# snakers4/mnasnet-pytorch

Hardware: AMD Instinct MI355X
Metric: images/sec MNASNet-1.0 224^2 bf16 train step (higher is better)
Workload: dtype bf16

## Files before the change

### mnasnet_pytorch_amd/csrc/mnas_tcx.hip

```cpp
#include "mnas_common.h"

struct TcxArgs {
    int M2;
    int Ho, Wo, Co, Ci;
    int Kpad;
    int rows_pad;
    int cib;
    float rcp_hw, rcp_wo;
    const uint16_t* dy;
    const uint16_t* w;
    void* out;
    float* stats;
    const void* red_y;
    const float* red_bn;
};

__device__ __forceinline__ int tcx_fdiv(int n, int d, float rcp) {
    if (rcp == 0.f) return n / d;
    int q = (int)((float)n * rcp);
    const int r = n - q * d;
    q += (r >= d) ? 1 : 0;
    q -= (r < 0) ? 1 : 0;
    return q;
}

template <int TPW, int KSM>
__global__ __launch_bounds__(256) void k_tcx(TcxArgs a) {
    extern __shared__ __attribute__((aligned(16))) unsigned char smem[];
    constexpr int WC = TPW * 16, SP = WC + 8;
    uint16_t* stage = (uint16_t*)smem;
    float* lds_rc = (float*)(stage + 4 * 16 * SP);
    float* lds_fin = lds_rc + 4 * WC;
    const int tid = threadIdx.x, lane = tid & 63;
    const int cls = __builtin_amdgcn_readfirstlane(tid >> 6);
    const int ph = cls >> 1, pw = cls & 1;
    const int l15 = lane & 15, lg = lane >> 4;
    const int ci0 = blockIdx.y * a.cib;
    const int cin = min(a.cib, a.Ci - ci0);
    const bool do_red = a.red_y != nullptr;
    const int nslots = (1 + ph) * (1 + pw);
    const int kc = nslots * a.Co;

    if (do_red)
        for (int i = tid; i < 4 * WC; i += 256) {
            const int r = i / WC, c = i - r * WC, cc = ci0 + c;
            float v = 0.f;
            if (c < cin) {
                if (r == 0) v = a.red_bn[cc];
                else if (r == 1) v = a.red_bn[a.Ci + cc];
                else if (r == 2) v = a.red_bn[6 * a.Ci + cc];
                else v = -a.red_bn[5 * a.Ci + cc] * a.red_bn[6 * a.Ci + cc];
            }
            lds_rc[i] = v;
        }
    int koff[KSM];
    unsigned nbits = 0;
    bf16x8_t wf[TPW][KSM];
#pragma unroll
    for (int ks = 0; ks < KSM; ++ks) {
        const int k = ks * 32 + lg * 8;
        const int slot = k / a.Co, co = k - slot * a.Co;
        const bool kok = k < kc;
        int dh = 0, dw = 0;
        if (kok) {
            if (ph && pw) { dh = slot >> 1; dw = slot & 1; }
            else if (ph) dh = slot;
            else if (pw) dw = slot;
        }
        koff[ks] = kok ? (dh * a.Wo + dw) * a.Co + co : -1;
        nbits |= (unsigned)(dh | (dw << 1)) << (2 * ks);
        const int col = (dh * 2 + dw) * a.Co + co;
#pragma unroll
        for (int t = 0; t < TPW; ++t) {
            const int rl = t * 16 + l15;
            const int row = cls * a.Ci + ci0 + rl;
            uint4 v = make_uint4(0, 0, 0, 0);
            if (kok && rl < cin && row < a.rows_pad) v = *(const uint4*)(a.w + (size_t)row * a.Kpad + col);
            wf[t][ks] = *(const bf16x8_t*)&v;
        }
    }
    if (do_red) __syncthreads();

    uint16_t* st = stage + cls * 16 * SP;
    const int hw = a.Ho * a.Wo;
    const int ngroups = (a.M2 + 15) >> 4;
    const int cpp = cin >> 3;
    constexpr int NPASS = (16 * (WC / 8) + 63) / 64;
    float r1[NPASS][8], r2[NPASS][8];
#pragma unroll
    for (int p = 0; p < NPASS; ++p)
#pragma unroll
        for (int j = 0; j < 8; ++j) { r1[p][j] = 0.f; r2[p][j] = 0.f; }

    uint4 v0[KSM];
    int ooff[NPASS], ooff_n[NPASS];
    uint4 yv[NPASS], yv_n[NPASS];
    auto issue = [&](int g) {
        const int m = g * 16 + l15;
        const bool mok = m < a.M2;
        const int n = mok ? tcx_fdiv(m, hw, a.rcp_hw) : 0, rem = m - n * hw;
        const int i = mok ? tcx_fdiv(rem, a.Wo, a.rcp_wo) : 0, j = rem - i * a.Wo;
        const uint16_t* base = a.dy + (size_t)(mok ? m : 0) * a.Co;
#pragma unroll
        for (int ks = 0; ks < KSM; ++ks) {
            const int dh = (nbits >> (2 * ks)) & 1, dw = (nbits >> (2 * ks + 1)) & 1;
            v0[ks] = make_uint4(0, 0, 0, 0);
            if (mok && koff[ks] >= 0 && i + dh < a.Ho && j + dw < a.Wo) v0[ks] = *(const uint4*)(base + koff[ks]);
        }
#pragma unroll
        for (int p = 0; p < NPASS; ++p) {
            const int q = p * 64 + lane;
            const int px = q / cpp, ch = q - px * cpp;
            const int mm = g * 16 + px;
            ooff_n[p] = -1;
            yv_n[p] = make_uint4(0, 0, 0, 0);
            if (q < 16 * cpp && mm < a.M2) {
                const int n2 = tcx_fdiv(mm, hw, a.rcp_hw), rem2 = mm - n2 * hw;
                const int i2 = tcx_fdiv(rem2, a.Wo, a.rcp_wo), j2 = rem2 - i2 * a.Wo;
                ooff_n[p] = ((n2 * 2 * a.Ho + 2 * i2 + ph) * (2 * a.Wo) + 2 * j2 + pw) * a.Ci + ci0 + ch * 8;
                if (do_red) yv_n[p] = *(const uint4*)((const uint16_t*)a.red_y + ooff_n[p]);
            }
        }
    };
    if ((int)blockIdx.x < ngroups) issue(blockIdx.x);
    for (int g = blockIdx.x; g < ngroups; g += gridDim.x) {
        const int m0 = g * 16;
        bf16x8_t bf[KSM];
#pragma unroll
        for (int ks = 0; ks < KSM; ++ks) bf[ks] = *(const bf16x8_t*)&v0[ks];
#pragma unroll
        for (int p = 0; p < NPASS; ++p) { ooff[p] = ooff_n[p]; yv[p] = yv_n[p]; }
        if (g + (int)gridDim.x < ngroups) issue(g + gridDim.x);
#pragma unroll
        for (int t = 0; t < TPW; ++t) {
            f32x4_t acc = (f32x4_t){0.f, 0.f, 0.f, 0.f};
#pragma unroll
            for (int ks = 0; ks < KSM; ++ks) acc = __builtin_amdgcn_mfma_f32_16x16x32_bf16(wf[t][ks], bf[ks], acc, 0, 0, 0);
            uint2 pk;
            pk.x = pack_bf16(acc[0], acc[1]);
            pk.y = pack_bf16(acc[2], acc[3]);
            *(uint2*)(st + l15 * SP + t * 16 + lg * 4) = pk;
        }
        __builtin_amdgcn_wave_barrier();
#pragma unroll
        for (int p = 0; p < NPASS; ++p) {
            const int q = p * 64 + lane;
            const int px = q / cpp, ch = q - px * cpp;
            if (ooff[p] >= 0) {
                const uint4 pk = *(const uint4*)(st + px * SP + ch * 8);
                st_u4((uint16_t*)a.out + ooff[p], pk, true);
                if (do_red) {
                    const uint32_t gu[4] = {pk.x, pk.y, pk.z, pk.w}, yu[4] = {yv[p].x, yv[p].y, yv[p].z, yv[p].w};
                    const int cl = ch * 8;
#pragma unroll
                    for (int jj = 0; jj < 4; ++jj)
                        mnas_red2(gu[jj], yu[jj], mnas_ld2(lds_rc + cl + 2 * jj), mnas_ld2(lds_rc + WC + cl + 2 * jj),
                                  mnas_ld2(lds_rc + 2 * WC + cl + 2 * jj), mnas_ld2(lds_rc + 3 * WC + cl + 2 * jj), &r1[p][2 * jj], &r2[p][2 * jj]);
                }
            }
        }
        __builtin_amdgcn_wave_barrier();
    }
    if (do_red && a.stats) {
        float* outp = a.stats;
        for (int p = 0; p < NPASS; ++p) {
            __syncthreads();
#pragma unroll
            for (int j = 0; j < 8; ++j) { lds_fin[tid * 16 + j] = r1[p][j]; lds_fin[tid * 16 + 8 + j] = r2[p][j]; }
            __syncthreads();
            for (int i = tid; i < 2 * cin; i += 256) {
                const int r = i / cin, c = i - r * cin, cc = c >> 3, j = c & 7;
                float v = 0.f;
                for (int th = 0; th < 256; ++th)
                    if (((p * 64 + (th & 63)) % cpp) == cc && p * 64 + (th & 63) < 16 * cpp) v += lds_fin[th * 16 + r * 8 + j];
                float* d = outp + ((size_t)r * a.Ci + ci0 + c) * gridDim.x + blockIdx.x;
                *d = (p == 0 ? 0.f : *d) + v;
            }
        }
    }
}

struct TcxPlan { int tpw, ksm, cib, nblocks; size_t lds; };

int mnas_tcx_enabled() {
    static int on = -1;
    if (on < 0) on = mnas_diag_env("MNAS_TCX", 1);
    return on;
}
static bool tcx_plan(int Ho, int Wo, int Co, int Ci, TcxPlan* p) {
    if (!mnas_tcx_enabled() || (Co & 7) || (Ci & 7) || Co < 8 || Ci < 8 || Ho < 1 || Wo < 1) return false;
    const int ksm = (4 * Co + 31) / 32;
    if (Ci <= 16 && ksm <= 3) { p->tpw = 1; p->ksm = 3; }
    else if (Ci <= 32 && ksm <= 5) { p->tpw = 2; p->ksm = 5; }
    else return false;
    p->cib = p->tpw * 16 < Ci ? p->tpw * 16 : Ci;
    p->nblocks = (Ci + p->cib - 1) / p->cib;
    const int wc = p->tpw * 16;
    p->lds = (size_t)4 * 16 * (wc + 8) * 2 + (size_t)4 * wc * 4 + (size_t)256 * 16 * 4;
    return true;
}
int mnas_tcx_ok(int Ho, int Wo, int Co, int Ci) {
    TcxPlan p;
    return tcx_plan(Ho, Wo, Co, Ci, &p) ? 1 : 0;
}
int mnas_tcx_parts(int N, int Ho, int Wo, int Co, int Ci) {
    TcxPlan p;
    if (!tcx_plan(Ho, Wo, Co, Ci, &p)) return -1;
    if ((long long)N * Ho * Wo * 4 * Ci > 0x7fffffff) return -1;
    const long long groups = ((long long)N * Ho * Wo + 15) / 16;
    static int wgs = -1;
    if (wgs < 0) wgs = mnas_diag_env("MNAS_TCX_WGS", 0);
    int want = (wgs > 0 ? wgs : (p.tpw == 1 ? 1024 : 768)) / p.nblocks;
    if (want < 64) want = 64;
    return (int)(groups < want ? groups : want);
}

int mnas_tcx_dgrad(const MnasTconvDgrad* c, void* stream) {
    TcxPlan p;
    const long long M2 = (long long)c->N * c->Ho * c->Wo;
    if (M2 * 4 * c->Ci > 0x7fffffff || !tcx_plan(c->Ho, c->Wo, c->Co, c->Ci, &p)) return MNAS_EINVAL;
    TcxArgs a;
    a.M2 = (int)M2; a.Ho = c->Ho; a.Wo = c->Wo; a.Co = c->Co; a.Ci = c->Ci;
    a.Kpad = (4 * c->Co + 31) / 32 * 32; a.rows_pad = (4 * c->Ci + 15) / 16 * 16; a.cib = p.cib;
    a.rcp_hw = M2 < (1 << 24) ? 1.0f / (float)(c->Ho * c->Wo) : 0.f;
    a.rcp_wo = M2 < (1 << 24) ? 1.0f / (float)c->Wo : 0.f;
    a.dy = (const uint16_t*)c->dy; a.w = (const uint16_t*)c->w; a.out = c->out; a.stats = c->stats;
    a.red_y = c->red_y; a.red_bn = c->red_bn;
    hipStream_t s = (hipStream_t)stream;
#define MNAS_TCX(T_, K_) \
    if (p.tpw == T_ && p.ksm == K_) { \
        hipLaunchKernelGGL((k_tcx<T_, K_>), dim3(c->nparts, p.nblocks), dim3(256), p.lds, s, a); \
        MNAS_CHECK_LAUNCH(); \
        return MNAS_OK; \
    }
    MNAS_TCX(1, 3) MNAS_TCX(2, 5)
#undef MNAS_TCX
    return MNAS_EINVAL;
}

struct TcrArgs {
    int N, Ho, Wo, Co, Ci;
    int Kpad, rows_pad;
    int LW, Cp;
    const uint16_t* dy;
    const uint16_t* w;
    void* out;
    float* stats;
    const void* red_y;
    const float* red_bn;
};

template <int KQ0, int KQ1, int KQ3>
__global__ __launch_bounds__(512) void k_tcr(TcrArgs a) {
    extern __shared__ __attribute__((aligned(16))) unsigned char smem[];
    constexpr int NB = 16, PPW = NB + 4, NSLOT = 256, MAXS = 6;
    constexpr int KQ[4] = {KQ0, KQ1, KQ1, KQ3};
    const int tid = threadIdx.x, lane = tid & 63;
    const int wave = __builtin_amdgcn_readfirstlane(tid >> 6);
    const int kq = wave & 3, phalf = wave >> 2;
    const int l15 = lane & 15, lg = lane >> 4;
    const int img_elems = ((a.Ho + 1) * a.LW * a.Cp + 7) & ~7;
    uint16_t* img = (uint16_t*)smem;
    float* part = (float*)(img + img_elems);
    float* lds_rc = part + 4 * NSLOT * PPW;
    float* lds_fin = part;
    const int ci0 = blockIdx.y * NB;
    const bool do_red = a.red_y != nullptr;
    const int npc = a.Ho * a.Wo;

    for (int i = tid; i < img_elems >> 3; i += 512) ((uint4*)img)[i] = make_uint4(0, 0, 0, 0);
    if (do_red)
        for (int i = tid; i < 4 * NB; i += 512) {
            const int r = i / NB, cc = ci0 + i % NB;
            float v = 0.f;
            if (cc < a.Ci) {
                if (r == 0) v = a.red_bn[cc];
                else if (r == 1) v = a.red_bn[a.Ci + cc];
                else if (r == 2) v = a.red_bn[6 * a.Ci + cc];
                else v = -a.red_bn[5 * a.Ci + cc] * a.red_bn[6 * a.Ci + cc];
            }
            lds_rc[i] = v;
        }
    bf16x8_t wf0[KQ0], wf1[KQ1], wf2[KQ1], wf3[KQ3];
    int to0[KQ0], to1[KQ1], to2[KQ1], to3[KQ3];
    auto load_class = [&](auto& wf, auto& to, int cls, int kqn) {
        const int ph = cls >> 1, pw = cls & 1;
        const int kc = (1 + ph) * (1 + pw) * a.Co;
#pragma unroll
        for (int j = 0; j < kqn; ++j) {
            const int k = (kq + 4 * j) * 32 + lg * 8;
            const bool kok = k < kc;
            const int slot = kok ? k / a.Co : 0, co = kok ? k - slot * a.Co : 0;
            int dh = 0, dw = 0;
            if (ph && pw) { dh = slot >> 1; dw = slot & 1; }
            else if (ph) dh = slot;
            else if (pw) dw = slot;
            to[j] = kok ? (dh * a.LW + dw) * a.Cp + co : -1;
            const int row = cls * a.Ci + ci0 + l15, col = (dh * 2 + dw) * a.Co + co;
            uint4 v = make_uint4(0, 0, 0, 0);
            if (kok && ci0 + l15 < a.Ci && row < a.rows_pad) v = *(const uint4*)(a.w + (size_t)row * a.Kpad + col);
            wf[j] = *(const bf16x8_t*)&v;
        }
    };
    load_class(wf0, to0, 0, KQ0); load_class(wf1, to1, 1, KQ1); load_class(wf2, to2, 2, KQ1); load_class(wf3, to3, 3, KQ3);
    int pbase[2];
#pragma unroll
    for (int t = 0; t < 2; ++t) {
        const int p = (phalf * 2 + t) * 16 + l15;
        const int pp = p < npc ? p : 0;
        const int i = pp / a.Wo, j = pp - i * a.Wo;
        pbase[t] = (i * a.LW + j) * a.Cp;
    }
    const int c4 = tid & 3, srow = tid >> 2;
    const int coe = ci0 + c4 * 4;
    float s1[4] = {0.f, 0.f, 0.f, 0.f}, s2[4] = {0.f, 0.f, 0.f, 0.f};
    const int co8 = a.Co >> 3, in_slots = npc * co8;
    uint4 vimg[MAXS];
    auto fetch = [&](int n) {
        const uint16_t* src = a.dy + (size_t)n * npc * a.Co;
#pragma unroll
        for (int j = 0; j < MAXS; ++j) {
            const int q = tid + 512 * j;
            vimg[j] = make_uint4(0, 0, 0, 0);
            if (q < in_slots) vimg[j] = *(const uint4*)(src + (size_t)q * 8);
        }
    };
    auto place = [&]() {
#pragma unroll
        for (int j = 0; j < MAXS; ++j) {
            const int q = tid + 512 * j;
            if (q >= in_slots) continue;
            const int pixq = q / co8, c8 = q - pixq * co8;
            const int iy = pixq / a.Wo, ix = pixq - iy * a.Wo;
            *(uint4*)(img + (iy * a.LW + ix) * a.Cp + c8 * 8) = vimg[j];
        }
    };
    __syncthreads();
    if ((int)blockIdx.x < a.N) { fetch(blockIdx.x); place(); }
    for (int n = blockIdx.x; n < a.N; n += gridDim.x) {
        __syncthreads();
        const int nn = n + gridDim.x;
        if (nn < a.N) fetch(nn);
        int ooff[2];
        uint2 ypre[2];
#pragma unroll
        for (int e = 0; e < 2; ++e) {
            const int slot = srow + 128 * e, cls = slot >> 6, p = slot & 63;
            ooff[e] = -1; ypre[e] = make_uint2(0, 0);
            if (p < npc && coe < a.Ci) {
                const int i = p / a.Wo, j = p - i * a.Wo;
                ooff[e] = (((n * 2 * a.Ho) + 2 * i + (cls >> 1)) * (2 * a.Wo) + 2 * j + (cls & 1)) * a.Ci + coe;
                if (do_red) ypre[e] = *(const uint2*)((const uint16_t*)a.red_y + ooff[e]);
            }
        }
        f32x4_t acc[4][2];
#pragma unroll
        for (int c = 0; c < 4; ++c)
#pragma unroll
            for (int t = 0; t < 2; ++t) acc[c][t] = (f32x4_t){0.f, 0.f, 0.f, 0.f};
        auto run_class = [&](const auto& wf, const auto& to, int cls, int kqn, f32x4_t (&ac)[2]) {
#pragma unroll
            for (int j = 0; j < kqn; ++j) {
#pragma unroll
                for (int t = 0; t < 2; ++t) {
                    uint4 bv = make_uint4(0, 0, 0, 0);
                    if (to[j] >= 0) bv = *(const uint4*)(img + pbase[t] + to[j]);
                    ac[t] = __builtin_amdgcn_mfma_f32_16x16x32_bf16(wf[j], *(const bf16x8_t*)&bv, ac[t], 0, 0, 0);
                }
            }
        };
        run_class(wf0, to0, 0, KQ0, acc[0]); run_class(wf1, to1, 1, KQ1, acc[1]);
        run_class(wf2, to2, 2, KQ1, acc[2]); run_class(wf3, to3, 3, KQ3, acc[3]);
#pragma unroll
        for (int c = 0; c < 4; ++c)
#pragma unroll
            for (int t = 0; t < 2; ++t)
                *(float4*)(part + ((size_t)kq * NSLOT + c * 64 + (phalf * 2 + t) * 16 + l15) * PPW + lg * 4) = *(const float4*)&acc[c][t];
        __syncthreads();
#pragma unroll
        for (int e = 0; e < 2; ++e) {
            if (ooff[e] < 0) continue;
            const int slot = srow + 128 * e;
            const float* src = part + (size_t)slot * PPW + c4 * 4;
            float4 v = *(const float4*)src;
#pragma unroll
            for (int q = 1; q < 4; ++q) {
                const float4 x = *(const float4*)(src + (size_t)q * NSLOT * PPW);
                v.x += x.x; v.y += x.y; v.z += x.z; v.w += x.w;
            }
            uint2 pk;
            pk.x = pack_bf16(v.x, v.y);
            pk.y = pack_bf16(v.z, v.w);
            *(uint2*)((uint16_t*)a.out + ooff[e]) = pk;
            if (do_red) {
                const int cl = c4 * 4;
                mnas_red2(pk.x, ypre[e].x, mnas_ld2(lds_rc + cl), mnas_ld2(lds_rc + NB + cl), mnas_ld2(lds_rc + 2 * NB + cl),
                          mnas_ld2(lds_rc + 3 * NB + cl), s1, s2);
                mnas_red2(pk.y, ypre[e].y, mnas_ld2(lds_rc + cl + 2), mnas_ld2(lds_rc + NB + cl + 2), mnas_ld2(lds_rc + 2 * NB + cl + 2),
                          mnas_ld2(lds_rc + 3 * NB + cl + 2), s1 + 2, s2 + 2);
            }
        }
        if (nn < a.N) place();
    }
    if (do_red && a.stats) {
        __syncthreads();
#pragma unroll
        for (int r = 0; r < 4; ++r) {
            lds_fin[(srow * 2 + 0) * NB + c4 * 4 + r] = s1[r];
            lds_fin[(srow * 2 + 1) * NB + c4 * 4 + r] = s2[r];
        }
        __syncthreads();
        for (int i = tid; i < 2 * NB; i += 512) {
            const int r = i / NB, cl = i - r * NB, cc = ci0 + cl;
            float v = lds_fin[r * NB + cl];
            for (int q = 1; q < 128; ++q) v += lds_fin[(q * 2 + r) * NB + cl];
            if (cc < a.Ci) a.stats[((size_t)r * a.Ci + cc) * gridDim.x + blockIdx.x] = v;
        }
    }
}

static bool tcr_plan(int Ho, int Wo, int Co, int Ci, int* parts_max, size_t* lds) {
    if (!mnas_tcx_enabled() || (Co & 31) || (Ci & 15) || Ho * Wo > 64 || Ho < 1 || Wo < 1) return false;
    if (Co != 192) return false;
    if ((long long)Co * Ci < 16 * 1024) return false;
    const size_t img = (((size_t)(Ho + 1) * (Wo + 1) * (Co + 8) + 7) & ~(size_t)7) * 2;
    *lds = img + (size_t)4 * 256 * 20 * 4 + (size_t)4 * 16 * 4;
    if ((size_t)Ho * Wo * (Co / 8) > 512 * 6 || *lds > 160 * 1024) return false;
    const int slices = Ci / 16;
    *parts_max = 256 / slices < 1 ? 1 : 256 / slices;
    return true;
}
int mnas_tcr_ok(int Ho, int Wo, int Co, int Ci) {
    int pm; size_t lds;
    return tcr_plan(Ho, Wo, Co, Ci, &pm, &lds) ? 1 : 0;
}
int mnas_tcr_parts(int N, int Ho, int Wo, int Co, int Ci) {
    int pm; size_t lds;
    if (N < 32 || !tcr_plan(Ho, Wo, Co, Ci, &pm, &lds)) return -1;
    if ((long long)N * 4 * Ho * Wo * Ci > 0x7fffffff) return -1;
    return pm < N ? pm : N;
}
int mnas_tcr_dgrad(const MnasTconvDgrad* c, void* stream) {
    int pm; size_t lds;
    if (c->N < 32 || !tcr_plan(c->Ho, c->Wo, c->Co, c->Ci, &pm, &lds)) return MNAS_EINVAL;
    if ((long long)c->N * 4 * c->Ho * c->Wo * c->Ci > 0x7fffffff) return MNAS_EINVAL;
    TcrArgs a;
    a.N = c->N; a.Ho = c->Ho; a.Wo = c->Wo; a.Co = c->Co; a.Ci = c->Ci;
    a.Kpad = (4 * c->Co + 31) / 32 * 32; a.rows_pad = (4 * c->Ci + 15) / 16 * 16;
    a.LW = c->Wo + 1; a.Cp = c->Co + 8;
    a.dy = (const uint16_t*)c->dy; a.w = (const uint16_t*)c->w; a.out = c->out; a.stats = c->stats;
    a.red_y = c->red_y; a.red_bn = c->red_bn;
    hipLaunchKernelGGL((k_tcr<2, 3, 6>), dim3(c->nparts, c->Ci / 16), dim3(512), lds, (hipStream_t)stream, a);
    MNAS_CHECK_LAUNCH();
    return MNAS_OK;
}
```

Before: 26240.

## Add row-paired transposed-conv dgrad kernel computing both column phases per wave

Adds k_tcw, a 128-thread transposed-conv dgrad kernel in which each wave handles one row phase and computes both column phases together. The paired outputs are staged into shared memory so stores are contiguous. It keeps multiple groups of loads in flight (D-deep prefetch), keeps BN reduce coefficients in registers for TPW=1, and gathers output bases with ds_bpermute. The TPW=1 path now uses the new kernel by default. The stats tail reduction in both kernels is replaced with a direct strided sum, and diagnostic ablation switches are added. The risks are extra padding MFMAs, higher register pressure, and a changed order of reduction summation.

```diff
diff --git a/mnasnet_pytorch_amd/csrc/mnas_tcx.hip b/mnasnet_pytorch_amd/csrc/mnas_tcx.hip
--- a/mnasnet_pytorch_amd/csrc/mnas_tcx.hip
+++ b/mnasnet_pytorch_amd/csrc/mnas_tcx.hip
@@ -13,7 +13,16 @@
     float* stats;
     const void* red_y;
     const float* red_bn;
+    int abl;
+    int long_tail;
 };
+#ifdef MNAS_DIAG
+#define TCX_ABL(a_) ((a_).abl)
+#define TCX_LONG_TAIL(a_) ((a_).long_tail)
+#else
+#define TCX_ABL(a_) 0
+#define TCX_LONG_TAIL(a_) 0
+#endif
 
 __device__ __forceinline__ int tcx_fdiv(int n, int d, float rcp) {
     if (rcp == 0.f) return n / d;
@@ -22,6 +31,222 @@
     q += (r >= d) ? 1 : 0;
     q -= (r < 0) ? 1 : 0;
     return q;
+}
+
+template <int TPW, int KS>
+__device__ __forceinline__ void tcw_class(const TcxArgs& a, int ph, int pw, int ci0, int cin, int l15, int lg, bf16x8_t (&wf)[TPW][KS],
+                                          int (&koff)[KS], unsigned& nbits) {
+    const int kc = (1 + ph) * (1 + pw) * a.Co;
+    nbits = 0;
+#pragma unroll
+    for (int ks = 0; ks < KS; ++ks) {
+        const int k = ks * 32 + lg * 8;
+        const int slot = k / a.Co, co = k - slot * a.Co;
+        const bool kok = k < kc;
+        int dh = 0, dw = 0;
+        if (kok) {
+            if (ph && pw) { dh = slot >> 1; dw = slot & 1; }
+            else if (ph) dh = slot;
+            else if (pw) dw = slot;
+        }
+        koff[ks] = kok ? (dh * a.Wo + dw) * a.Co + co : -1;
+        nbits |= (unsigned)(dh | (dw << 1)) << (2 * ks);
+        const int col = (dh * 2 + dw) * a.Co + co;
+#pragma unroll
+        for (int t = 0; t < TPW; ++t) {
+            const int rl = t * 16 + l15;
+            const int row = (ph * 2 + pw) * a.Ci + ci0 + rl;
+            uint4 v = make_uint4(0, 0, 0, 0);
+            if (kok && rl < cin && row < a.rows_pad) v = *(const uint4*)(a.w + (size_t)row * a.Kpad + col);
+            wf[t][ks] = *(const bf16x8_t*)&v;
+        }
+    }
+}
+
+__device__ const uint4 tcw_zero16 = {0u, 0u, 0u, 0u};
+
+typedef __bf16 tcw_bf2 __attribute__((ext_vector_type(2)));
+typedef float tcw_f2 __attribute__((ext_vector_type(2)));
+__device__ __forceinline__ uint32_t tcw_pack(float lo, float hi) {
+    const tcw_bf2 r = __builtin_convertvector((tcw_f2){lo, hi}, tcw_bf2);
+    return *(const uint32_t*)&r;
+}
+
+template <int TPW, int KSA, int KSB, int D>
+__global__ __launch_bounds__(128, 2) void k_tcw(TcxArgs a) {
+    extern __shared__ __attribute__((aligned(16))) unsigned char smem[];
+    constexpr int WC = TPW * 16, SP = WC + 8;
+    constexpr int NPASS = (32 * (WC / 8) + 63) / 64;
+    static_assert(16 * (WC / 8) <= 64, "k_tcx's copy-out role map (one pass per class) is what the reduce's order is kept against");
+    uint16_t* stage = (uint16_t*)smem;
+    float* lds_rc = (float*)(stage + 2 * 32 * SP);
+    float* lds_fin = lds_rc + 4 * WC;
+    const int tid = threadIdx.x, lane = tid & 63;
+    const int ph = __builtin_amdgcn_readfirstlane(tid >> 6);
+    const int l15 = lane & 15, lg = lane >> 4;
+    const int ci0 = blockIdx.y * a.cib;
+    const int cin = min(a.cib, a.Ci - ci0);
+    const bool do_red = a.red_y != nullptr;
+
+    if (do_red)
+        for (int i = tid; i < 4 * WC; i += 128) {
+            const int r = i / WC, c = i - r * WC, cc = ci0 + c;
+            float v = 0.f;
+            if (c < cin) {
+                if (r == 0) v = a.red_bn[cc];
+                else if (r == 1) v = a.red_bn[a.Ci + cc];
+                else if (r == 2) v = a.red_bn[6 * a.Ci + cc];
+                else v = -a.red_bn[5 * a.Ci + cc] * a.red_bn[6 * a.Ci + cc];
+            }
+            lds_rc[i] = v;
+        }
+    int koffa[KSA], koffb[KSB];
+    unsigned nbitsa, nbitsb;
+    bf16x8_t wfa[TPW][KSA], wfb[TPW][KSB];
+    tcw_class<TPW, KSA>(a, ph, 0, ci0, cin, l15, lg, wfa, koffa, nbitsa);
+    tcw_class<TPW, KSB>(a, ph, 1, ci0, cin, l15, lg, wfb, koffb, nbitsb);
+    if (do_red) __syncthreads();
+
+    uint16_t* st = stage + ph * 32 * SP;
+    const int hw = a.Ho * a.Wo;
+    const int ngroups = (a.M2 + 15) >> 4;
+    const int cpp = cin >> 3;
+    float r1[NPASS][8], r2[NPASS][8];
+#pragma unroll
+    for (int p = 0; p < NPASS; ++p)
+#pragma unroll
+        for (int j = 0; j < 8; ++j) { r1[p][j] = 0.f; r2[p][j] = 0.f; }
+    int co_o[NPASS], co_ch[NPASS], co_add[NPASS];
+#pragma unroll
+    for (int p = 0; p < NPASS; ++p) {
+        const int c = p * 64 + lane;
+        co_o[p] = c < 32 * cpp ? c / cpp : -1;
+        co_ch[p] = c - (c / cpp) * cpp;
+        co_add[p] = (co_o[p] & 1) * a.Ci + co_ch[p] * 8;
+    }
+    constexpr bool RCREG = TPW == 1;
+    mnas_f2 rc[RCREG ? NPASS : 1][4][4];
+    if (RCREG && do_red) {
+#pragma unroll
+        for (int p = 0; p < NPASS; ++p)
+#pragma unroll
+            for (int r = 0; r < 4; ++r)
+#pragma unroll
+                for (int jj = 0; jj < 4; ++jj) rc[p][r][jj] = mnas_ld2(lds_rc + r * WC + co_ch[p] * 8 + 2 * jj);
+    }
+
+    uint4 va[D][KSA], vb[D][KSB];
+    int ooff[D][NPASS];
+    uint4 yv[D][NPASS];
+    auto issue = [&](int d, int g) {
+        const int m = g * 16 + l15;
+        const bool mok = m < a.M2;
+        const int n = mok ? tcx_fdiv(m, hw, a.rcp_hw) : 0, rem = m - n * hw;
+        const int i = mok ? tcx_fdiv(rem, a.Wo, a.rcp_wo) : 0, j = rem - i * a.Wo;
+        const uint16_t* base = a.dy + (size_t)(mok ? m : 0) * a.Co;
+        const uint16_t* zero = (const uint16_t*)&tcw_zero16;
+#pragma unroll
+        for (int ks = 0; ks < KSA; ++ks) {
+            const int dh = (nbitsa >> (2 * ks)) & 1, dw = (nbitsa >> (2 * ks + 1)) & 1;
+            const bool ok = mok && koffa[ks] >= 0 && i + dh < a.Ho && j + dw < a.Wo;
+            va[d][ks] = *(const uint4*)(ok ? base + koffa[ks] : zero);
+        }
+#pragma unroll
+        for (int ks = 0; ks < KSB; ++ks) {
+            const int dh = (nbitsb >> (2 * ks)) & 1, dw = (nbitsb >> (2 * ks + 1)) & 1;
+            const bool ok = mok && koffb[ks] >= 0 && i + dh < a.Ho && j + dw < a.Wo;
+            vb[d][ks] = *(const uint4*)(ok ? base + koffb[ks] : zero);
+        }
+        const int obase = mok ? ((n * 2 * a.Ho + 2 * i + ph) * (2 * a.Wo) + 2 * j) * a.Ci + ci0 : -1;
+#pragma unroll
+        for (int p = 0; p < NPASS; ++p) {
+            const int ob = __builtin_amdgcn_ds_bpermute((co_o[p] >> 1) << 2, obase);
+            const bool ok = co_o[p] >= 0 && ob >= 0;
+            const int o = ob + co_add[p];
+            ooff[d][p] = ok ? o : -1;
+            yv[d][p] = make_uint4(0, 0, 0, 0);
+            if (do_red && !(TCX_ABL(a) & 2)) yv[d][p] = *(const uint4*)((const uint16_t*)a.red_y + (ok ? o : 0));
+        }
+    };
+    const bf16x8_t zf = {0, 0, 0, 0, 0, 0, 0, 0};
+    const int gstep = gridDim.x;
+#pragma unroll
+    for (int d = 0; d < D; ++d)
+        if ((int)blockIdx.x + d * gstep < ngroups) issue(d, blockIdx.x + d * gstep);
+    for (int g0 = blockIdx.x; g0 < ngroups; g0 += D * gstep) {
+#pragma unroll
+        for (int d = 0; d < D; ++d) {
+            const int g = g0 + d * gstep;
+            if (g >= ngroups) continue;
+            bf16x8_t bfa[KSA], bfb[KSB];
+#pragma unroll
+            for (int ks = 0; ks < KSA; ++ks) bfa[ks] = *(const bf16x8_t*)&va[d][ks];
+#pragma unroll
+            for (int ks = 0; ks < KSB; ++ks) bfb[ks] = *(const bf16x8_t*)&vb[d][ks];
+#pragma unroll
+            for (int t = 0; t < TPW; ++t) {
+                f32x4_t acca = (f32x4_t){0.f, 0.f, 0.f, 0.f}, accb = (f32x4_t){0.f, 0.f, 0.f, 0.f};
+#pragma unroll
+                for (int ks = 0; ks < KSA; ++ks) acca = __builtin_amdgcn_mfma_f32_16x16x32_bf16(wfa[t][ks], bfa[ks], acca, 0, 0, 0);
+#pragma unroll
+                for (int ks = KSA; ks < KSB; ++ks) acca = __builtin_amdgcn_mfma_f32_16x16x32_bf16(zf, zf, acca, 0, 0, 0);
+#pragma unroll
+                for (int ks = 0; ks < KSB; ++ks) accb = __builtin_amdgcn_mfma_f32_16x16x32_bf16(wfb[t][ks], bfb[ks], accb, 0, 0, 0);
+                uint2 pk;
+                pk.x = tcw_pack(acca[0], acca[1]);
+                pk.y = tcw_pack(acca[2], acca[3]);
+                *(uint2*)(st + (2 * l15) * SP + t * 16 + lg * 4) = pk;
+                pk.x = tcw_pack(accb[0], accb[1]);
+                pk.y = tcw_pack(accb[2], accb[3]);
+                *(uint2*)(st + (2 * l15 + 1) * SP + t * 16 + lg * 4) = pk;
+            }
+            __builtin_amdgcn_wave_barrier();
+#pragma unroll
+            for (int p = 0; p < NPASS; ++p) {
+                if (ooff[d][p] >= 0) {
+                    const uint4 pk = *(const uint4*)(st + co_o[p] * SP + co_ch[p] * 8);
+                    if (!(TCX_ABL(a) & 1)) st_u4((uint16_t*)a.out + ooff[d][p], pk, true);
+                    if (do_red) {
+                        const uint32_t gu[4] = {pk.x, pk.y, pk.z, pk.w}, yu[4] = {yv[d][p].x, yv[d][p].y, yv[d][p].z, yv[d][p].w};
+                        const int cl = co_ch[p] * 8;
+#pragma unroll
+                        for (int jj = 0; jj < 4; ++jj) {
+                            if (RCREG)
+                                mnas_red2(gu[jj], yu[jj], rc[p][0][jj], rc[p][1][jj], rc[p][2][jj], rc[p][3][jj], &r1[p][2 * jj], &r2[p][2 * jj]);
+                            else
+                                mnas_red2(gu[jj], yu[jj], mnas_ld2(lds_rc + cl + 2 * jj), mnas_ld2(lds_rc + WC + cl + 2 * jj),
+                                          mnas_ld2(lds_rc + 2 * WC + cl + 2 * jj), mnas_ld2(lds_rc + 3 * WC + cl + 2 * jj), &r1[p][2 * jj], &r2[p][2 * jj]);
+                        }
+                    }
+                }
+            }
+            __builtin_amdgcn_wave_barrier();
+            if (g + D * gstep < ngroups) issue(d, g + D * gstep);
+        }
+    }
+    if (do_red && a.stats) {
+        __syncthreads();
+#pragma unroll
+        for (int p = 0; p < NPASS; ++p)
+            if (co_o[p] >= 0) {
+                const int th = (2 * ph + (co_o[p] & 1)) * 64 + (co_o[p] >> 1) * cpp + co_ch[p];
+#pragma unroll
+                for (int j = 0; j < 8; ++j) { lds_fin[th * 16 + j] = r1[p][j]; lds_fin[th * 16 + 8 + j] = r2[p][j]; }
+            }
+        __syncthreads();
+        for (int i = tid; i < 2 * cin; i += 128) {
+            const int r = i / cin, c = i - r * cin, cc = c >> 3, j = c & 7;
+            float v = 0.f;
+            for (int cls = 0; cls < 4; ++cls) {
+                float e[16];
+#pragma unroll
+                for (int px = 0; px < 16; ++px) e[px] = lds_fin[(cls * 64 + px * cpp + cc) * 16 + r * 8 + j];
+#pragma unroll
+                for (int px = 0; px < 16; ++px) v += e[px];
+            }
+            a.stats[((size_t)r * a.Ci + ci0 + c) * gridDim.x + blockIdx.x] = v;
+        }
+    }
 }
 
 template <int TPW, int KSM>
@@ -118,7 +343,7 @@
                 const int n2 = tcx_fdiv(mm, hw, a.rcp_hw), rem2 = mm - n2 * hw;
                 const int i2 = tcx_fdiv(rem2, a.Wo, a.rcp_wo), j2 = rem2 - i2 * a.Wo;
                 ooff_n[p] = ((n2 * 2 * a.Ho + 2 * i2 + ph) * (2 * a.Wo) + 2 * j2 + pw) * a.Ci + ci0 + ch * 8;
-                if (do_red) yv_n[p] = *(const uint4*)((const uint16_t*)a.red_y + ooff_n[p]);
+                if (do_red && !(TCX_ABL(a) & 2)) yv_n[p] = *(const uint4*)((const uint16_t*)a.red_y + ooff_n[p]);
             }
         }
     };
@@ -148,7 +373,7 @@
             const int px = q / cpp, ch = q - px * cpp;
             if (ooff[p] >= 0) {
                 const uint4 pk = *(const uint4*)(st + px * SP + ch * 8);
-                st_u4((uint16_t*)a.out + ooff[p], pk, true);
+                if (!(TCX_ABL(a) & 1)) st_u4((uint16_t*)a.out + ooff[p], pk, true);
                 if (do_red) {
                     const uint32_t gu[4] = {pk.x, pk.y, pk.z, pk.w}, yu[4] = {yv[p].x, yv[p].y, yv[p].z, yv[p].w};
                     const int cl = ch * 8;
@@ -171,8 +396,18 @@
             for (int i = tid; i < 2 * cin; i += 256) {
                 const int r = i / cin, c = i - r * cin, cc = c >> 3, j = c & 7;
                 float v = 0.f;
-                for (int th = 0; th < 256; ++th)
-                    if (((p * 64 + (th & 63)) % cpp) == cc && p * 64 + (th & 63) < 16 * cpp) v += lds_fin[th * 16 + r * 8 + j];
+                if (NPASS == 1 && !TCX_LONG_TAIL(a)) {
+                    for (int cls = 0; cls < 4; ++cls) {
+                        float e[16];
+#pragma unroll
+                        for (int px = 0; px < 16; ++px) e[px] = lds_fin[(cls * 64 + px * cpp + cc) * 16 + r * 8 + j];
+#pragma unroll
+                        for (int px = 0; px < 16; ++px) v += e[px];
+                    }
+                } else {
+                    for (int th = 0; th < 256; ++th)
+                        if (((p * 64 + (th & 63)) % cpp) == cc && p * 64 + (th & 63) < 16 * cpp) v += lds_fin[th * 16 + r * 8 + j];
+                }
                 float* d = outp + ((size_t)r * a.Ci + ci0 + c) * gridDim.x + blockIdx.x;
                 *d = (p == 0 ? 0.f : *d) + v;
             }
@@ -226,15 +461,32 @@
     a.rcp_wo = M2 < (1 << 24) ? 1.0f / (float)c->Wo : 0.f;
     a.dy = (const uint16_t*)c->dy; a.w = (const uint16_t*)c->w; a.out = c->out; a.stats = c->stats;
     a.red_y = c->red_y; a.red_bn = c->red_bn;
+    a.abl = mnas_diag_env("MNAS_TCX_ABL", 0);
     hipStream_t s = (hipStream_t)stream;
+    int row = p.tpw == 1 ? 1 : 3;
+#ifdef MNAS_DIAG
+    row = mnas_diag_env("MNAS_TCX_ROW", row);
+#endif
+    a.long_tail = row == 0;
+    row = row == 1;
 #define MNAS_TCX(T_, K_) \
-    if (p.tpw == T_ && p.ksm == K_) { \
+    if (!row && p.tpw == T_ && p.ksm == K_) { \
         hipLaunchKernelGGL((k_tcx<T_, K_>), dim3(c->nparts, p.nblocks), dim3(256), p.lds, s, a); \
         MNAS_CHECK_LAUNCH(); \
         return MNAS_OK; \
     }
-    MNAS_TCX(1, 3) MNAS_TCX(2, 5)
+#define MNAS_TCW(T_, KA_, KB_, D_) \
+    if (row && p.tpw == T_ && p.ksm == KB_) { \
+        hipLaunchKernelGGL((k_tcw<T_, KA_, KB_, D_>), dim3(c->nparts, p.nblocks), dim3(128), p.lds, s, a); \
+        MNAS_CHECK_LAUNCH(); \
+        return MNAS_OK; \
+    }
+    MNAS_TCW(1, 2, 3, 3) MNAS_TCX(2, 5)
+#ifdef MNAS_DIAG
+    MNAS_TCX(1, 3) MNAS_TCW(2, 3, 5, 2)
+#endif
 #undef MNAS_TCX
+#undef MNAS_TCW
     return MNAS_EINVAL;
 }
 
```

Measured after the change: 26350 (median of 6 runs). Within noise of the previous version (+0.4%).
